# utiasSTARS/pyslam

Hardware: AMD Instinct MI355X
Metric: ms/LM-iter (Jac build + J^T J + Schur solve), stereo BA @ 500k residuals (lower is better)
Workload: dtype f64

## Files before the change

### pyslam_amd/csrc/ps_abi_problem.h

```cpp


const char* ps_last_error(void) { return g_err.c_str(); }

int ps_device_count(void) {
    int n = 0;
    if (hipGetDeviceCount(&n) != hipSuccess) return 0;
    return n;
}

int ps_warm_up(void) {
    static std::once_flag once;
    static int rc = 0;
    std::call_once(once, [] {
        void* p = nullptr;
        if (hipMalloc(&p, 256) != hipSuccess) { rc = fail("hipMalloc failed (no usable HIP device?)"); return; }
        hipLaunchKernelGGL(k_zero4, dim3(1), dim3(256), 0, 0, (size_t)8, (double*)p, (size_t)0, (double*)nullptr, (size_t)0,
                           (double*)nullptr, (size_t)0, (double*)nullptr);
        double hostw[4] = {0, 0, 0, 0};
        (void)hipMemsetAsync(p, 0, 256, 0);
        (void)hipMemcpyAsync((char*)p + 128, p, 64, hipMemcpyDeviceToDevice, 0);
        (void)hipMemcpyAsync(hostw, p, sizeof(hostw), hipMemcpyDeviceToHost, 0);
        if (hipDeviceSynchronize() != hipSuccess) rc = fail("the warm-up launch failed");
        hipFree(p);
        hipFuncAttributes a;
#define PS_TOUCH(...) (void)hipFuncGetAttributes(&a, reinterpret_cast<const void*>(&__VA_ARGS__))
        PS_TOUCH(k_landmark_pass<false>); PS_TOUCH(k_landmark_pass_packed<false, false>); PS_TOUCH(k_landmark_pass_packed<false, true>); PS_TOUCH(k_backsub_packed<false>); PS_TOUCH(k_pose_pass<false>); PS_TOUCH(k_pose_finalize); PS_TOUCH(k_schur_pairs_db<0>);
        PS_TOUCH(k_schur_combine); PS_TOUCH(k_backsub<false>); PS_TOUCH(k_cost_reproj<false>); PS_TOUCH(k_cost_packed<false>); PS_TOUCH(k_reduce3); PS_TOUCH(k_reduce_partials);
        PS_TOUCH(k_copy2); PS_TOUCH(k_zero4); PS_TOUCH(k_lag_status_check);
        PS_TOUCH(k_block_jacobi_factor<6>); PS_TOUCH(k_scale_blocks<6>); PS_TOUCH(k_scale_blocks_p<6>); PS_TOUCH(k_rows_setup<6>);
        PS_TOUCH(k_coarse_rowsums<6>); PS_TOUCH(k_coarse_matrix<6>); PS_TOUCH(k_coarse_chol<6, true>); PS_TOUCH(k_coarse_border<6>);
        PS_TOUCH(k_coarse_mreduce<6>); PS_TOUCH(k_coarse_xbuild<6>); PS_TOUCH(k_coarse_recover<6>); PS_TOUCH(k_cg_fused_lds<6, 8>);
        PS_TOUCH(k_cg_fused<6, 8>); PS_TOUCH(k_cg_unscale<6>); PS_TOUCH(k_update_poses<6>); PS_TOUCH(k_update_points);
        PS_TOUCH(k_xcoarse_rowsums<6>); PS_TOUCH(k_xcoarse_matrix<6>); PS_TOUCH(k_band_chol<6>); PS_TOUCH(k_band_inverse); PS_TOUCH(k_band_inverse_rl<false>);
        PS_TOUCH(k_band_inverse_rl<true>); PS_TOUCH(k_bp_v); PS_TOUCH(k_bp_t); PS_TOUCH(k_bp_w); PS_TOUCH(k_bp_dense_sep); PS_TOUCH(k_bp_dense);
        PS_TOUCH(k_xcg_restrict<6>); PS_TOUCH(k_xcg_f2_coarse<6, 3>); PS_TOUCH(k_xcg_fused1<6, 8, false>); PS_TOUCH(k_xcg_fused1<6, 0, true>);
        PS_TOUCH(k_xcg_fused1<6, 2, false>); PS_TOUCH(k_xcg_fused1<6, 6, false>);
        PS_TOUCH(k_factor_pass<6>); PS_TOUCH(k_factor_assemble<6>); PS_TOUCH(k_cost_factors<6>);
        PS_TOUCH(k_factor_pass<3>); PS_TOUCH(k_factor_assemble<3>); PS_TOUCH(k_cost_factors<3>); PS_TOUCH(k_block_jacobi_factor<3>);
        PS_TOUCH(k_update_poses<3>); PS_TOUCH(k_direct_solve<6>); PS_TOUCH(k_direct_solve<3>);
        PS_TOUCH(k_motion_only_solve<false>); PS_TOUCH(k_motion_only_iteration<false>);
        PS_TOUCH(k_pcg_spmv<6>); PS_TOUCH(k_pcg_spmv<3>); PS_TOUCH(k_ldi_init); PS_TOUCH(k_ldi_update); PS_TOUCH(k_ldi_gemm); PS_TOUCH(k_ldi_mirror);
        PS_TOUCH(k_ldi_ritz); PS_TOUCH(k_ldi_seed_prep); PS_TOUCH(k_ldi_fro_total); PS_TOUCH(k_ldi_pad_identity);
        PS_TOUCH(k_ldi_scaled_dense<6>); PS_TOUCH(k_ldi_sym_unscale<6>); PS_TOUCH(k_ldi_scaled_dense<3>); PS_TOUCH(k_ldi_sym_unscale<3>);
        PS_TOUCH(k_shard_pack<6>); PS_TOUCH(k_shard_unpack<6>); PS_TOUCH(k_publish); PS_TOUCH(k_cov_rhs); PS_TOUCH(k_triangulate<false>);
        PS_TOUCH(k_scale_blocks<3>); PS_TOUCH(k_rows_setup<3>); PS_TOUCH(k_coarse_rowsums<3>); PS_TOUCH(k_coarse_matrix<3>);
        PS_TOUCH(k_coarse_chol<3, true>); PS_TOUCH(k_coarse_border<3>); PS_TOUCH(k_coarse_mreduce<3>); PS_TOUCH(k_coarse_xbuild<3>);
        PS_TOUCH(k_coarse_recover<3>); PS_TOUCH(k_cg_fused_lds<3, 8>); PS_TOUCH(k_cg_unscale<3>);
#undef PS_TOUCH
    });
// ... 574 lines not shown
        row_ptr[a + 1]++;
        if (a != b) row_ptr[b + 1]++;
    }
    for (int r = 0; r < nr; ++r) row_ptr[r + 1] += row_ptr[r];
    const long nnzb_l = row_ptr[nr];
    if (nnzb_l * DD >= (1L << 31)) return fail("reduced system too large for 32-bit block offsets");
    const int nnzb = h->nnzb = (int)nnzb_l;
    col_idx.assign(nnzb, 0);
    {
        std::vector<int32_t> f2(row_ptr.begin(), row_ptr.end() - 1);
        for (uint64_t k : keys) { const int a = (int)(k >> 32), b = (int)(uint32_t)k; if (a != b) col_idx[f2[b]++] = a; }
        for (uint64_t k : keys) { const int a = (int)(k >> 32), b = (int)(uint32_t)k; col_idx[f2[a]++] = b; }
    }
    auto slot_of = [&](int a, int b) -> int {
        const int32_t* lo = col_idx.data() + row_ptr[a];
        const int32_t* hi = col_idx.data() + row_ptr[a + 1];
        const int32_t* it = std::lower_bound(lo, hi, b);
        return (it != hi && *it == b) ? (int)(it - col_idx.data()) : -1;
    };
    std::vector<int32_t> diag_slot(nr);
    for (int r = 0; r < nr; ++r) diag_slot[r] = slot_of(r, r);
    if (h->upload(&h->row_ptr, row_ptr) || h->upload(&h->col_idx, col_idx) || h->upload(&h->diag_slot, diag_slot)) return -1;
    h->red_count = (long)nnzb * DD + (long)nr * D + 2;
    if (h->alloc(&h->red, (size_t)h->red_count + ST_NWORDS / 2)) return -1;
    h->status = reinterpret_cast<int32_t*>(h->red + h->red_count);
    h->S = h->red; h->g = h->red + (size_t)nnzb * DD; h->red_cost = h->g + (size_t)nr * D;

    lap("block pattern");
    std::vector<PairItem> pitm(task_start.size());
    {
        const long nt = (long)pitm.size();
        std::atomic<int> diag{0};
        ps_parallel(ps_host_threads(nt * 16), [&](int t, int TT) {
            for (long q = nt * t / TT, e = nt * (t + 1) / TT; q < e; ++q) {
                const uint64_t key = task_keyv[q];
                const int a = (int)(key >> 32), b = (int)(uint32_t)key;
                pitm[q] = {slot_of(a, b), slot_of(b, a), task_start[q], q + 1 < nt ? task_start[q + 1] : (int32_t)npairs_l};
                if (a == b) diag = 1;
            }
        });
        if (diag) h->has_diag_tasks = true;
    }
    h->npair_items = (int)pitm.size();
    if (!dev_pairs && h->upload(&h->pairs, pairs)) return -1;
    {
        std::vector<std::vector<int32_t>> lists(8);
        const double total = (double)npairs_l;
        for (size_t k = 0; k < pitm.size(); ++k) {
// ... 193 lines not shown
```

### pyslam_amd/csrc/ps_abi_solver.h

```cpp

int ps_get_info(ps_problem* h, ps_problem_info* info) {
    if (!h || !info) return fail("null argument");
    info->dof = h->D; info->num_poses = h->P; info->num_reduced = h->nr; info->num_points = h->L;
    info->num_var_points = h->nv; info->num_obs = h->N; info->num_edges = h->F; info->num_priors = 0;
    info->reduced_nnzb = h->nnzb; info->num_pairs = h->npairs;
    info->reduce_count = ((long)h->nnzb + h->nr) / 2 * h->D * h->D + (long)h->nr * h->D + 3;
    info->device_bytes = (int64_t)h->dev_bytes;
    info->cg_restarts = h->cg_fallbacks;
    info->cg_kernel_launches = h->cg_kernel_launches;
    info->ldi_solves = h->ldi_solves; info->ldi_fallbacks = h->ldi_fallbacks; info->ldi_seeds = h->ldi_seeds;
    info->xcg_fused_solves = h->xf_solves; info->xcg_fused_fallbacks = h->xf_fallbacks;
    info->cg_persist_solves = h->cp_launches; info->cg_persist_failures = h->cp_failures;
    info->cg_persist_refused = h->cp_refused; info->persist_cus = h->persist_cus;
    info->persist_cus_needed = h->cp_ok ? h->cp_cus_needed : (h->xp_ok ? h->xp_cus_needed : 0);
    info->landmark_passes_taken_over = h->prelm_used;
    return 0;
}

int ps_eval_cost(ps_problem* h, int include_all_constant, double* cost) {
    if (!h || !cost) return fail("null argument");
    if (include_all_constant && h->fuse_cost == 1 && lm_cost_possible(h)) { if (lm_cost_pass(h, h->lin_lambda, SC_COST)) return -1; }
    else if (cost_pass(h, include_all_constant, SC_COST)) return -1;
    if (read_scalars(h)) return -1;
    *cost = h->h_scalars[SC_COST];
// ... 810 lines not shown
    if (n == "solve_horizon") { h->solve_horizon = value < 0 ? -1 : (int)std::min(value, 1e6); return 0; }
    h->prelin_valid = h->prelm_valid = false;
    if (n == "pcg_variant") { if (value != 0 && value != 1) return fail("pcg_variant must be 0 or 1"); h->pcg_variant = (int)value; }
    else if (n == "coarse_groups") {
        if (value < -1 || value >= PS_XCG_MAXNODES) return fail("coarse_groups out of range (-1 auto, 0 off, else number of hat intervals; above 63 only for the explicit two-level PCG, at most 1023)");
        h->coarse_req = (int)value; h->coarse_built = false;
    }
#ifdef PS_MEASURE
    else if (n == "cg_ablate") h->cg_ablate = (int)value;
    else if (n == "schur_ablate") h->schur_ablate = (int)value;
    else if (n == "lm_ablate") h->lm_ablate = (int)value;
#else
    else if (n == "cg_ablate" || n == "schur_ablate" || n == "lm_ablate") {
        if (value != 0.0) return fail(n + ": timing experiments exist in the measurement build only (__graft_entry__.build_measure(), PYSLAM_AMD_MEASURE=1)");
    }
#endif
    else if (n == "schur_pipeline") h->schur_pipeline = value != 0.0;
    else if (n == "coarse_lag") h->coarse_lag = value != 0.0;
    else if (n == "cg_force_restart") h->cg_force_restart = value != 0.0;
    else if (n == "xcg_restrict_fused") h->xcg_rt = value != 0;
    else if (n == "band_chol") { h->band_chol = value != 0; h->lci_next = -1; }
    else if (n == "lm_packed") h->lm_packed = value != 0;
    else if (n == "pose_xcd") h->pose_xcd = value != 0;
    else if (n == "fuse_cost") h->fuse_cost = (int)value;
    else if (n == "sync_refactor") h->sync_refactor = value != 0;
    else if (n == "hold_across_steps") h->hold_across_steps = value != 0;
    else if (n == "band_part") { h->band_part = value != 0; h->lci_next = -1; }
    else if (n == "band_part_chunk") { if (value < 0 || value > 4096) return fail("band_part_chunk must be 0 (automatic) .. 4096 nodes"); h->band_part_m = (int)value; h->lci_next = -1; }
    else if (n == "coarse_auto_hold") h->xcg_auto_hold = value != 0;
    else if (n == "coarse_adaptive_hold") h->xcg_adaptive_hold = value != 0;
    else if (n == "xcg_fused") { if (value != 0 && value != 1 && value != 2) return fail("xcg_fused must be 0, 1 or 2"); h->xcg_fused = (int)value; }
    else if (n == "lagged_inverse") { h->ldi_enable = value != 0; if (!h->ldi_enable) { h->ldi_cur = -1; if (h->ldi_state != 1) h->ldi_state = 0; } relook_path(h); }
    else if (n == "ldi_max_unknowns") { if (value < 0 || value > PS_LDI_MAXN) return fail("ldi_max_unknowns out of range (0 .. 3328)"); h->ldi_max_n = (int)value; relook_path(h); }
    else if (n == "ldi_cap") { if (value < 1 || value > 64) return fail("ldi_cap out of range (1 .. 64)"); h->ldi_cap = (int)value; }
    else if (n == "ldi_cost_tol") { if (!(value >= 0)) return fail("ldi_cost_tol must be >= 0"); h->ldi_cost_tol = value; }
    else if (n == "ldi_refresh_its") { if (value < 0 || value > 64) return fail("ldi_refresh_its out of range (0 .. 64)"); h->ldi_refresh_its = (int)value; }
    else if (n == "ldi_direct") { h->ldi_direct_ok = value != 0.0; h->ldi_direct = value > 0.0; }
    else if (n == "direct_fused") h->direct_fused = value != 0.0;
    else if (n == "ldi_seed_lag") { if (value < 1 || value > 16) return fail("ldi_seed_lag out of range (1 .. 16)"); h->ldi_seed_lag = (int)value; }
    else if (n == "ldi_seed_steps") { if (value < 1 || value > 40) return fail("ldi_seed_steps out of range (1 .. 40)"); h->ldi_seed_steps = (int)value; }
    else if (n == "coarse_refresh_every") { if (value < 1 || value > 16) return fail("coarse_refresh_every must be 1..16"); h->xcg_refresh_every = (int)value; }
    else if (n == "coarse_lag_x") { h->lagx = value != 0.0; h->lci_next = -1; h->side_todo = false; }
    else if (n == "cg_lds") h->cg_lds = value != 0.0;
    else if (n == "cg_persist") h->cg_persist = value != 0.0;
    else if (n == "xcg_persist") h->xcg_persist = value != 0.0;
    else if (n == "cg_persist_spin") { if (value < 0 || value > 1e7) return fail("cg_persist_spin out of range"); h->cp_spin = (unsigned)value; }
// ... 101 lines not shown
```

### pyslam_amd/csrc/ps_core.hip

```cpp
#include <hip/hip_runtime.h>

#include <algorithm>
#include <array>
#include <map>
#include <atomic>
#include <chrono>
#include <thread>
#include <climits>
#include <cmath>
#include <cstdio>
#include <cstring>
#include <memory>
#include <mutex>
#include <string>
#include <vector>

#include "pyslam_hip.h"
#include "ps_kernels.h"
#include "ps_ransac.h"
#include "ps_k_twoview.h"
#include "ps_photo.h"
#include "ps_k_dense.h"
#include "ps_k_feat.h"
#include "ps_sparse.h"
// ... 326 lines not shown
    typedef int (*allreduce_fn)(const void*, void*, size_t, int, int, void*, hipStream_t);
    allreduce_fn nccl_allreduce = nullptr;
    void* nccl_comm = nullptr;
    typedef int (*allgather_fn)(const void*, void*, size_t, int, void*, hipStream_t);
    allgather_fn seg_allgather = nullptr;
    int seg_world = 0, seg_rank = 0;
    long seg_maxlen = 0, seg_nmine = 0, seg_ndst = 0;
    int32_t *seg_mine = nullptr, *seg_dst = nullptr, *seg_src_off = nullptr, *seg_src_ptr = nullptr;
    double *seg_in = nullptr, *seg_all = nullptr;
    double* shard_pack = nullptr;
    int32_t *up_slot = nullptr, *upT_slot = nullptr;
    long nup = 0, pack_count = 0;
    double* shard_buf = nullptr;
    bool shard_out = false;
    double *sq_part_l = nullptr, *sq_part_p = nullptr;
    bool lm_md = false;
    double *md_part_p = nullptr, *md_part_l = nullptr;
    int nmd_p = 0;
    int nsq_l = 0 , nsq_l16 = 0 , nsq_p = 0;
    int32_t* lmw_first = nullptr;
    int lmw_nwaves = 0;
    int lm_packed = 1;
    int pose_xcd = 1;
    int ldi_enable = 1;
    int ldi_max_n = 2048;
    int ldi_cap = 12;
    int ldi_seed_steps = 3;
    double ldi_cost_tol = 0.05;
    bool ldi_ready = false;
    int ldi_n = 0, ldi_np = 0, ldi_kp = 0;
    float *ldi_S32 = nullptr, *ldi_X32 = nullptr, *ldi_R32 = nullptr, *ldi_T32 = nullptr, *ldi_Xt = nullptr, *ldi_XtT = nullptr;
    float* ldi_Xu[2] = {};
    double *ldi_x64 = nullptr, *ldi_Linv = nullptr, *ldi_r[2] = {}, *ldi_part = nullptr, *ldi_fro_part = nullptr;
    double *h_ldi_fro = nullptr, *h_ldi_fro_dev = nullptr;
    int ldi_state = 0;
    int ldi_cur = -1, ldi_next = -1;
    long ldi_iter = 0, ldi_ready_at = 0;
    double ldi_fro_limit = 0.1, ldi_last_rms = 0.0;
    bool ldi_side_todo = false, ldi_update_ok = false, ldi_sread_pending = false, ldi_ritz_ok = false;
    double ldi_ritz_lo = 0.0, ldi_ritz_hi = 0.0;
    int ldi_last_its = 0, ldi_prev_its = 0;
    int ldi_refresh_its = 7;
    bool ldi_refreshed = false;
    int2* ldi_krange = nullptr;
    int ldi_seed_lag = ps_env("PS_LDI_SEED_LAG") ? atoi(ps_env("PS_LDI_SEED_LAG")) : 1;
    int ldi_rejects = 0; long ldi_no_seed_before = 0;
// ... 168 lines not shown
```

### pyslam_amd/csrc/ps_host_cg.h

```cpp

namespace {

struct StageTimer {
    ps_problem* h;
    int stage;
    hipEvent_t a = nullptr, b = nullptr;
    int slot = -1;
    StageTimer(ps_problem* h_, int st, int level = 2) : h(h_), stage(st) {
        if (h->profiling < level) return;
        if (h->profiling == 1 && h->prof_every > 1 &&
            h->prof_tick % h->prof_every != (st == PS_ST_CG_KERNEL ? h->prof_every / 2 : 0)) return;
        if (h->ev_used + 2 > h->ev_pool.size()) {
            for (int i = 0; i < 64; ++i) { hipEvent_t e; hipEventCreate(&e); h->ev_pool.push_back(e); }
        }
        slot = (int)h->ev_used;
        a = h->ev_pool[h->ev_used++];
        b = h->ev_pool[h->ev_used++];
        hipEventRecord(a, h->stream);
    }
    void stop() {
        if (!a) return;
        hipEventRecord(b, h->stream);
        h->pending.push_back({stage, slot});
        a = nullptr;
// ... 848 lines not shown
    if (iters_out) *iters_out = total_its;
    if (relres_out) *relres_out = rel * reduced;
    h->last_pcg_iters = total_its;
    return rc;
}

int linearize(ps_problem* h, double lambda, bool allow_prelm) {
    h->solver_touched = true;
    h->prelin_valid = false;
    const bool lm_done = allow_prelm && h->prelm_valid && h->prelm_lambda == lambda && h->nv > 0;
    h->prelm_valid = false;
    h->lin_lmfail_tag = lm_done ? h->prelm_tag : 0;
    if (lm_done) ++h->prelm_used;
    h->lin_lambda = lambda;
    h->params_moved_since_lin = false; h->z_foreign = false;
    ++h->prof_tick;
    h->cov_ready = false;
    cov_release(h);
    h->status_clean = false;
    if (h->ldi_sread_pending) {
        HIP_OK(hipStreamWaitEvent(h->stream, h->ev_ldi_sread, 0));
        h->ldi_sread_pending = false;
    }
    HIP_OK(hipMemsetAsync(h->red, 0, h->red_count * sizeof(double) + ST_NWORDS * sizeof(int32_t), h->stream));
    if (h->nv > 0 && !lm_done) {
        StageTimer t(h, PS_ST_LANDMARK);
        const ObsWide wl{h->sidx_l, h->stiff_tab};
#define PS_LM_LAUNCH(W) hipLaunchKernelGGL(k_landmark_pass<W>, dim3(cdiv(h->nv, 256 / PS_LM_GROUP)), dim3(256), 0, h->stream, h->nv, h->lm_ptr, \
                           h->lm_point, h->lobs, h->poses, h->points, h->pose_rid, h->ogroups, lambda, h->Z,                       \
                           h->Cinv, h->cvec, h->status, h->lm_ablate, wl)
#define PS_LMP_LAUNCH(W) hipLaunchKernelGGL((k_landmark_pass_packed<W, false>), dim3(cdiv(h->lmw_nwaves, 4)), dim3(256), 0, h->stream, h->lmw_nwaves, \
                           h->lmw_first, h->lm_ptr, h->lm_point, h->lobs, h->poses, h->points, h->pose_rid, h->ogroups, lambda, h->Z,      \
                           h->Cinv, h->cvec, h->status, wl, (const int32_t*)nullptr, (double*)nullptr, (long long*)nullptr, 0LL)
        if (h->lm_packed && h->lmw_nwaves > 0 && !h->lm_ablate) { if (h->wide_obs) PS_LMP_LAUNCH(true); else PS_LMP_LAUNCH(false); }
        else if (h->wide_obs) PS_LM_LAUNCH(true); else PS_LM_LAUNCH(false);
#undef PS_LMP_LAUNCH
#undef PS_LM_LAUNCH
    }
    bool fin_in_combine = false, fin_in_pairs = false;
    static const bool schur_split_env = ps_env("PS_SCHUR_SPLIT") != nullptr;
    if (h->npitems > 0) {
        StageTimer t(h, PS_ST_POSE);
        const ObsWide wp{h->sidx_p, h->stiff_tab};
        const int per_xcd = h->pose_xcd ? cdiv(h->npitems, 8) : 0;
        const int nblk = per_xcd ? 8 * per_xcd : h->npitems;
        if (h->wide_obs)
            hipLaunchKernelGGL(k_pose_pass<true>, dim3(nblk), dim3(256), 0, h->stream, h->pitems, h->pobs,
                               h->poses, h->points, h->ogroups, h->Cinv, h->cvec, h->ppartial, lambda != 0.0 ? 1 : 0, wp, h->npitems, per_xcd);
        else
            hipLaunchKernelGGL(k_pose_pass<false>, dim3(nblk), dim3(256), 0, h->stream, h->pitems, h->pobs,
                               h->poses, h->points, h->ogroups, h->Cinv, h->cvec, h->ppartial, lambda != 0.0 ? 1 : 0, wp, h->npitems, per_xcd);
        fin_in_combine = h->Spart && h->npair_items > 0 && !h->has_diag_tasks && h->D == 6;
        fin_in_pairs = !h->Spart && h->schur_pipeline && h->npair_items > 0 && !h->has_diag_tasks && h->D == 6 && !schur_split_env;
        if (!fin_in_combine && !fin_in_pairs)
            hipLaunchKernelGGL(k_pose_finalize, dim3(h->nr), dim3(64), 0, h->stream, h->nr, h->pitem_ptr,
                               h->ppartial, h->diag_slot, lambda, h->S, h->g);
    }
    if (h->npair_items > 0) {
        StageTimer t(h, PS_ST_SCHUR, 1);
        const bool split2 = schur_split_env;
        const int halfp = split2 ? (h->pair_per_xcd / 2 + 3) / 4 * 4 : h->pair_per_xcd;
        static const int lds_pad = ps_env("PS_SCHUR_LDS_PAD") ? atoi(ps_env("PS_SCHUR_LDS_PAD")) : 0;
        auto launch_pairs = [&](int nblk, int lds, int from, int to) {
            if (!h->schur_pipeline)
                hipLaunchKernelGGL(k_schur_pairs, dim3(nblk), dim3(256), lds, h->stream, h->pair_per_xcd, h->pair_xitems, h->pairs,
                                   h->Z, h->S, h->Spart, h->schur_ablate, from, to);
            else {
#ifdef PS_MEASURE
                auto k = h->schur_ablate == 0 ? k_schur_pairs_db<0> : h->schur_ablate == 1 ? k_schur_pairs_db<1> :
                         h->schur_ablate == 2 ? k_schur_pairs_db<2> : h->schur_ablate == 3 ? k_schur_pairs_db<3> :
                         h->schur_ablate == 4 ? k_schur_pairs_db<4> : k_schur_pairs_db<5>;
#else
                auto k = k_schur_pairs_db<0>;
#endif
                hipLaunchKernelGGL(k, dim3(nblk + (fin_in_pairs ? cdiv(h->nr, 4) : 0)), dim3(256), lds, h->stream, h->pair_per_xcd,
                                   h->pair_xitems, h->pairs, h->Z, h->S, h->Spart, from, to, nblk, fin_in_pairs ? h->nr : 0,
                                   h->pitem_ptr, h->ppartial, h->diag_slot, lambda, h->g);
            }
        };
        launch_pairs(8 * (halfp / 4), lds_pad, 0, halfp);
        if (split2 && halfp < h->pair_per_xcd) launch_pairs(8 * ((h->pair_per_xcd - halfp + 3) / 4), 0, halfp, h->pair_per_xcd);
        if (h->Spart)
            hipLaunchKernelGGL(k_schur_combine, dim3(cdiv(h->ncomb, 4) + (fin_in_combine ? cdiv(h->nr, 4) : 0)), dim3(256), 0,
                               h->stream, h->ncomb, h->comb_items, h->comb_tasks, h->Spart, h->S,
                               fin_in_combine ? h->nr : 0, h->pitem_ptr, h->ppartial, h->diag_slot, lambda, h->g);
    }
    if ((h->F > 0 || h->FH > 0) && h->nr > 0) {
        StageTimer t(h, PS_ST_EDGES);
        if (h->D == 6) launch_factor_pass<6>(h, lambda); else launch_factor_pass<3>(h, lambda);
    }
    return side_kick(h);
}

inline bool cost_packed_possible(const ps_problem* h) {
    return h->fuse_cost != 0 && h->lm_packed && h->lmw_nwaves > 0 && !h->lm_ablate && h->Nl == h->N && h->nv > 0 && h->D == 6;
}
int cost_partials_pass(ps_problem* h, int include_all, const int32_t* gate) {
    int n = 0;
    if (h->N > 0 && include_all && cost_packed_possible(h)) {
        const ObsWide wl{h->sidx_l, h->stiff_tab};
// ... 193 lines not shown
```

### pyslam_amd/csrc/ps_k_linearize.h

```cpp
#pragma once

#define PS_LM_GROUP 16

PS_DEV double group16_sum(double v) {
    v = dpp_shift_add<0x111, 0xf, 0xf>(v);
    v = dpp_shift_add<0x112, 0xf, 0xf>(v);
    v = dpp_shift_add<0x114, 0xf, 0xe>(v);
    v = dpp_shift_add<0x118, 0xf, 0xc>(v);
    return __shfl(v, (int)(threadIdx.x & 63) | 15, 64);
}

#define PS_ZROW 16

PS_DEV void lm_emit_m(const ReprojEval& ev, double M00, double M10, double M11, double M20, double M21,
                      double M22, double* __restrict__ m) {
#pragma unroll
    for (int a = 0; a < 3; ++a) {
        const double w0 = ev.Jp[a] * ev.Jl[0] + ev.Jp[6 + a] * ev.Jl[3] + ev.Jp[12 + a] * ev.Jl[6];
        const double w1 = ev.Jp[a] * ev.Jl[1] + ev.Jp[6 + a] * ev.Jl[4] + ev.Jp[12 + a] * ev.Jl[7];
        const double w2 = ev.Jp[a] * ev.Jl[2] + ev.Jp[6 + a] * ev.Jl[5] + ev.Jp[12 + a] * ev.Jl[8];
        m[3 * a] = w0 * M00;
        m[3 * a + 1] = w0 * M10 + w1 * M11;
        m[3 * a + 2] = w0 * M20 + w1 * M21 + w2 * M22;
    }
// ... 145 lines not shown
        F[i][2] = E[i][1] * x - E[i][0] * y;
    }
    acc[0] += e[0]; acc[1] += e[1]; acc[2] += e[2]; acc[3] += F[0][0]; acc[4] += F[0][1]; acc[5] += F[0][2];
    acc[6] += e[3]; acc[7] += e[4]; acc[8] += F[1][0]; acc[9] += F[1][1]; acc[10] += F[1][2];
    acc[11] += e[5]; acc[12] += F[2][0]; acc[13] += F[2][1]; acc[14] += F[2][2];
    acc[15] += y * F[2][0] - z * F[1][0];
    acc[16] += y * F[2][1] - z * F[1][1];
    acc[17] += y * F[2][2] - z * F[1][2];
    acc[18] += z * F[0][1] - x * F[2][1];
    acc[19] += z * F[0][2] - x * F[2][2];
    acc[20] += x * F[1][2] - y * F[0][2];
}

#define PS_NPOSE_ACC 33
#ifndef PS_POSE_TRANSPOSE
#define PS_POSE_TRANSPOSE 1
#endif
typedef const __attribute__((address_space(1))) void* ps_gptr_t;
typedef __attribute__((address_space(3))) void* ps_lptr_t;

#ifndef PS_POSE_WAVES
#define PS_POSE_WAVES 3
#endif
template <bool WIDE>
__global__ __launch_bounds__(256) __attribute__((amdgpu_waves_per_eu(PS_POSE_WAVES, 8))) void k_pose_pass(
    const PItem* __restrict__ items,
    const LObs* __restrict__ pobs ,
    const double* __restrict__ poses, const double* __restrict__ points,
    const ObsGroup* __restrict__ groups, const double* __restrict__ Cinv,
    const double* __restrict__ cvec, double* __restrict__ partial, int want_diag ,
    ObsWide wide, int nitems, int per_xcd )
{
    __shared__ double red[4][PS_NPOSE_ACC];
#if PS_POSE_TRANSPOSE
    __shared__ double tr[4][64 * 17];
#endif
    const int item = per_xcd > 0 ? (int)(blockIdx.x & 7) * per_xcd + (int)(blockIdx.x >> 3) : (int)blockIdx.x;
    if (item >= nitems) return;
    const PItem it = items[item];
    const int w = threadIdx.x >> 6, lane = threadIdx.x & 63;
    const Se3 T = se3_load(poses + 12 * (size_t)it.pad);
    double acc[PS_NPOSE_ACC];
#pragma unroll
    for (int k = 0; k < PS_NPOSE_ACC; ++k) acc[k] = 0.0;
    for (int i = it.start + threadIdx.x; i < it.end; i += 256) {
        const LObs o = pobs[i];
        const int v = PS_POSE_OF(o) - 1;
        const double pw[3] = {points[3 * (size_t)o.point], points[3 * (size_t)o.point + 1], points[3 * (size_t)o.point + 2]};
        double m[6] = {0, 0, 0, 0, 0, 0}, c0 = 0.0, c1 = 0.0, c2 = 0.0;
        if (v >= 0) {
            const double* ci = Cinv + 6 * (size_t)v;
#pragma unroll
            for (int k = 0; k < 6; ++k) m[k] = ci[k];
            c0 = cvec[3 * (size_t)v]; c1 = cvec[3 * (size_t)v + 1]; c2 = cvec[3 * (size_t)v + 2];
        }
        ReprojEval ev;
        reproj_eval_obs<true, true, WIDE>(T, pw, &o.u, groups, PS_GRP_OF(o), wide, i, ev);
        double G[6], t3[3];
        {
            const double* J = ev.Jp;
            G[0] = J[0] * J[0] + J[6] * J[6] + J[12] * J[12];
// ... 12 lines not shown
            pose_sandwich(G, ev.pc, d21);
            acc[27] += d21[0]; acc[28] += d21[6]; acc[29] += d21[11]; acc[30] += d21[15]; acc[31] += d21[18]; acc[32] += d21[20];
        }
        if (v >= 0) {
            double m9[9];
            lm_emit_m(ev, m[0], m[1], m[2], m[3], m[4], m[5], m9);
            G[0] -= m9[0] * m9[0] + m9[1] * m9[1] + m9[2] * m9[2];
            G[1] -= m9[0] * m9[3] + m9[1] * m9[4] + m9[2] * m9[5];
            G[2] -= m9[0] * m9[6] + m9[1] * m9[7] + m9[2] * m9[8];
            G[3] -= m9[3] * m9[3] + m9[4] * m9[4] + m9[5] * m9[5];
            G[4] -= m9[3] * m9[6] + m9[4] * m9[7] + m9[5] * m9[8];
            G[5] -= m9[6] * m9[6] + m9[7] * m9[7] + m9[8] * m9[8];
#pragma unroll
            for (int a = 0; a < 3; ++a) t3[a] += m9[3 * a] * c0 + m9[3 * a + 1] * c1 + m9[3 * a + 2] * c2;
        }
        pose_sandwich(G, ev.pc, acc);
        acc[21] -= t3[0]; acc[22] -= t3[1]; acc[23] -= t3[2];
        acc[24] -= ev.pc[1] * t3[2] - ev.pc[2] * t3[1];
        acc[25] -= ev.pc[2] * t3[0] - ev.pc[0] * t3[2];
        acc[26] -= ev.pc[0] * t3[1] - ev.pc[1] * t3[0];
    }
#if PS_POSE_TRANSPOSE
    {
        double* trw = tr[w];
#pragma unroll
        for (int h2 = 0; h2 < 2; ++h2) {
            const int k0 = 17 * h2, nk = h2 ? PS_NPOSE_ACC - 17 : 17;
#pragma unroll
            for (int k = 0; k < 17; ++k) if (k < nk) trw[lane * 17 + k] = acc[k0 + k];
            __builtin_amdgcn_wave_barrier();
            if (lane < nk) {
                double s = 0.0;
#pragma unroll 8
                for (int l = 0; l < 64; ++l) s += trw[l * 17 + lane];
                red[w][k0 + lane] = s;
            }
            __builtin_amdgcn_wave_barrier();
        }
    }
#else
#pragma unroll
    for (int k = 0; k < PS_NPOSE_ACC; ++k) {
        const double s = wave_sum(acc[k]);
        if (lane == 0) red[w][k] = s;
    }
#endif
    __syncthreads();
    if (threadIdx.x < PS_NPOSE_ACC)
        partial[(size_t)item * PS_NPOSE_ACC + threadIdx.x] =
            ((red[0][threadIdx.x] + red[1][threadIdx.x]) + red[2][threadIdx.x]) + red[3][threadIdx.x];
}

PS_DEV void pose_finalize_wave(int rid, int lane, const int32_t* __restrict__ pitem_ptr,
                               const double* __restrict__ partial, const int32_t* __restrict__ diag_slot,
                               double lambda, double* __restrict__ S, double* __restrict__ g, double* v )
{
    if (lane < PS_NPOSE_ACC) {
        double s = 0.0;
        for (int it = pitem_ptr[rid]; it < pitem_ptr[rid + 1]; ++it) s += partial[(size_t)it * PS_NPOSE_ACC + lane];
        v[lane] = s;
    }
    __builtin_amdgcn_wave_barrier();
    if (lane < 36) {
        const int r = lane / 6, c = lane % 6;
        const int a = r < c ? r : c, b = r < c ? c : r;
        const int idx = a * 6 - (a * (a - 1)) / 2 + (b - a);
        double val = v[idx];
        if (r == c) val += lambda * v[27 + r];
        S[(size_t)diag_slot[rid] * 36 + lane] += val;
    }
    if (lane < 6) g[(size_t)rid * 6 + lane] += v[21 + lane];
}

// ... 268 lines not shown
```

### pyslam_amd/csrc/ps_k_schur2.h

```cpp
#pragma once

#define PS_SQ_ROWD 12
#define PS_SQ_BUF (64 * PS_SQ_ROWD)
#define PS_SQ_BUFSTEP (4 * PS_SQ_BUF * 8)

typedef double ps_d2 __attribute__((ext_vector_type(2)));
#ifndef PS_SQ_ASM_CLOBBER
#define PS_SQ_ASM_CLOBBER "memory"
#endif

PS_DEV void sq_fetch_idx(const int32_t* __restrict__ src , int32_t* slot ) {
    __builtin_amdgcn_global_load_lds((ps_gptr_t)src, (ps_lptr_t)slot, 4, 0, 0);
}

template <bool HOT >
PS_DEV void sq_fetch(const double* __restrict__ Z, const uint32_t (&ia)[6], uint32_t slot_off, double* buf, const int (&off_of)[6]) {
    int zr[6];
    asm volatile(
        "ds_read_b32 %0, %6\n\t"
        "ds_read_b32 %1, %7\n\t"
        "ds_read_b32 %2, %8\n\t"
        "ds_read_b32 %3, %9\n\t"
        "ds_read_b32 %4, %10\n\t"
        "ds_read_b32 %5, %11\n\t"
// ... 38 lines not shown
#pragma unroll
        for (int k = 0; k < 9; ++k) A[k] = hf ? A[k] : ma[k];
    }
    double mb[12];
#pragma unroll
    for (int k = 0; k < 6; ++k) { mb[2 * k] = vb[k].x; mb[2 * k + 1] = vb[k].y; }
#pragma unroll
    for (int a = 0; a < 3; ++a)
#pragma unroll
        for (int b = 0; b < 3; ++b)
            acc[6 * a + b] += A[3 * a] * mb[3 * b] + A[3 * a + 1] * mb[3 * b + 1] + A[3 * a + 2] * mb[3 * b + 2];
    double Lb[9];
    zrow_cross(mb, mb + 9, Lb);
#pragma unroll
    for (int a = 0; a < 3; ++a)
#pragma unroll
        for (int b = 0; b < 3; ++b)
            acc[6 * a + 3 + b] += A[3 * a] * Lb[3 * b] + A[3 * a + 1] * Lb[3 * b + 1] + A[3 * a + 2] * Lb[3 * b + 2];
}

#define PS_SQ_WAIT_CHUNK() __builtin_amdgcn_s_waitcnt(0x0F70 | 7)
#define PS_SQ_WAIT_ALL() __builtin_amdgcn_s_waitcnt(0x0F70)

template <int ABL >
__global__ __launch_bounds__(256) __attribute__((amdgpu_waves_per_eu(3, 3))) void k_schur_pairs_db(
    int per_xcd, const PairItem* __restrict__ xitems, const int2* __restrict__ pairs, const double* __restrict__ Z,
    double* __restrict__ S, double* __restrict__ Spart, int first, int last,
    int fin_first_block, int fin_nr, const int32_t* __restrict__ pitem_ptr, const double* __restrict__ ppartial,
    const int32_t* __restrict__ diag_slot, double lambda, double* __restrict__ g)
{
    constexpr int ablate = ABL;
    __shared__ __attribute__((aligned(16))) double sbuf[2 * 4 * PS_SQ_BUF];
    __shared__ __attribute__((aligned(16))) int32_t sidx[4 * 256];
    const int lane = threadIdx.x & 63, wv = threadIdx.x >> 6;
    double* const buf0 = sbuf + wv * PS_SQ_BUF;
    double* const buf1 = buf0 + 4 * PS_SQ_BUF;
    int32_t* const islot = sidx + wv * 256;
    if ((int)blockIdx.x >= fin_first_block) {
        const int rid = ((int)blockIdx.x - fin_first_block) * 4 + wv;
        if (rid < fin_nr) pose_finalize_wave(rid, lane, pitem_ptr, ppartial, diag_slot, lambda, S, g, buf0);
        return;
    }
    const int local = first + (blockIdx.x >> 3) * 4 + wv;
    if (local >= last) return;
    const size_t pos = (size_t)(blockIdx.x & 7) * per_xcd + local;
    PairItem it = xitems[pos];
    it.slot = __builtin_amdgcn_readfirstlane(it.slot); it.slotT = __builtin_amdgcn_readfirstlane(it.slotT);
    it.start = __builtin_amdgcn_readfirstlane(it.start); it.end = __builtin_amdgcn_readfirstlane(it.end);
    if (it.slot < 0) return;
    const int p = lane & 31, hf = lane >> 5;
    const int32_t* flat = reinterpret_cast<const int32_t*>(pairs) + hf;
    uint32_t ia[6];
    int off_of[6];
#pragma unroll
    for (int k = 0; k < 6; ++k) {
        const int q = 64 * k + lane, row = q / 6;
        ia[k] = (uint32_t)(uintptr_t)(ps_lptr_t)(islot + row);
        off_of[k] = 2 * (q - 6 * row);
    }
    const uint32_t aa = (uint32_t)(uintptr_t)(ps_lptr_t)(buf0 + PS_SQ_ROWD * p), ab = aa + 32 * PS_SQ_ROWD * 8;
    double acc[18];
#pragma unroll
    for (int k = 0; k < 18; ++k) acc[k] = 0.0;
    const int npairs = it.end - it.start, nch = (npairs + 31) >> 5, last_pair = max(it.end - 1, 0);
#define PS_SQ_IDX(c) (flat + 2 * (size_t)min(it.start + 32 * (c) + p, last_pair))
    sq_fetch_idx(PS_SQ_IDX(0), islot + 0);
    sq_fetch_idx(PS_SQ_IDX(1), islot + 64);
    sq_fetch_idx(PS_SQ_IDX(2), islot + 128);
    PS_SQ_WAIT_ALL();
    __builtin_amdgcn_wave_barrier();
    if (!(ablate & 2)) sq_fetch<(ABL & 4) != 0>(Z, ia, 0, buf0, off_of);
    sq_fetch_idx(PS_SQ_IDX(3), islot + 192);
    if (nch > 1 && !(ablate & 2)) sq_fetch<(ABL & 4) != 0>(Z, ia, 256, buf1, off_of);
    int c = 0;
    for (; c + 2 < nch; ++c) {
        const uint32_t boff = (c & 1) * PS_SQ_BUFSTEP;
        PS_SQ_WAIT_CHUNK();
        __builtin_amdgcn_wave_barrier();
        if (!(ablate & 1)) sq_products(aa + boff, ab + boff, hf, acc);
        __builtin_amdgcn_wave_barrier();
        sq_fetch_idx(PS_SQ_IDX(c + 4), islot + 64 * (c & 3));
        if (!(ablate & 2)) sq_fetch<(ABL & 4) != 0>(Z, ia, 256 * ((c + 2) & 3), (c & 1) ? buf1 : buf0, off_of);
    }
    if (c + 1 < nch) {
        PS_SQ_WAIT_CHUNK();
        __builtin_amdgcn_wave_barrier();
        if (!(ablate & 1)) sq_products(aa + (c & 1) * PS_SQ_BUFSTEP, ab + (c & 1) * PS_SQ_BUFSTEP, hf, acc);
        __builtin_amdgcn_wave_barrier();
        ++c;
    }
    {
        PS_SQ_WAIT_ALL();
        __builtin_amdgcn_wave_barrier();
        if (p < npairs - 32 * c && !(ablate & 1)) sq_products(aa + (c & 1) * PS_SQ_BUFSTEP, ab + (c & 1) * PS_SQ_BUFSTEP, hf, acc);
        __builtin_amdgcn_wave_barrier();
    }
#undef PS_SQ_IDX
    double* sums = buf0;
#pragma unroll
    for (int k = 0; k < 18; ++k) {
        const double t = half_sum_dpp(acc[k]);
        if (p == 31) sums[18 * hf + k] = t;
    }
    __builtin_amdgcn_wave_barrier();
    if (lane < 36) {
// ... 13 lines not shown
```

### pyslam_amd/csrc/ps_kernels.h

```cpp
#pragma once
#include "ps_math.h"

struct __attribute__((aligned(32))) LObs {
    double u, v, d;
    int32_t pose_grp;
    int32_t point;
};
struct PItem { int32_t rid, start, end, pad; };
struct PairItem { int32_t slot, slotT, start, end; };
struct FactorGroup { double S[36]; int32_t loss_id; int32_t pad; double loss_k; };

#define PS_POSE_OF(o) ((o).pose_grp & 0xFFFFFF)
#define PS_GRP_OF(o) (((uint32_t)(o).pose_grp) >> 24)

enum { ST_LM_FAIL = 0, ST_DIAG_FAIL = 1, ST_PCG_DONE = 2, ST_PCG_ITERS = 3, ST_PERSIST_FAIL = 4 , ST_NWORDS = 8 };
enum { SC_COST = 0, SC_DXP2 = 1, SC_LINCOST = 2, SC_RR0 = 3, SC_RRFINAL = 4, SC_THRESH = 5, SC_DXL2 = 6, SC_STARTCOST = 7, SC_MODELDEC = 8, SC_NWORDS = 9 };

template <int CTRL, int ROW_MASK, int BANK_MASK>
PS_DEV double dpp_shift_add(double v) {
    const unsigned long long b = __builtin_bit_cast(unsigned long long, v);
    const int lo = __builtin_amdgcn_update_dpp(0, (int)(unsigned)b, CTRL, ROW_MASK, BANK_MASK, false);
    const int hi = __builtin_amdgcn_update_dpp(0, (int)(unsigned)(b >> 32), CTRL, ROW_MASK, BANK_MASK, false);
    const unsigned long long m = ((unsigned long long)(unsigned)hi << 32) | (unsigned)lo;
    return v + __builtin_bit_cast(double, m);
// ... 52 lines not shown
```

Baseline: 0.3062.

## Merge pose linearization pass into Schur pair kernel with atomic arrival finalize

Pose-pass workgroups now run inside the Schur pair kernel launch, reusing its LDS. The last workgroup to finish a pose row, detected through a per-row atomic arrival counter, runs the pose finalize for that row. This removes one kernel launch and the stream serialization between the pose pass and the pair pass, letting the two phases overlap. In exchange it adds atomics, memory fences and an extra zeroed counter array, and the pose work may now compete with the pair work for occupancy under the pair kernel's waves-per-EU limit.

```diff
diff --git a/pyslam_amd/csrc/ps_abi_problem.h b/pyslam_amd/csrc/ps_abi_problem.h
--- a/pyslam_amd/csrc/ps_abi_problem.h
+++ b/pyslam_amd/csrc/ps_abi_problem.h
@@ -24,7 +24,7 @@
         hipFree(p);
         hipFuncAttributes a;
 #define PS_TOUCH(...) (void)hipFuncGetAttributes(&a, reinterpret_cast<const void*>(&__VA_ARGS__))
-        PS_TOUCH(k_landmark_pass<false>); PS_TOUCH(k_landmark_pass_packed<false, false>); PS_TOUCH(k_landmark_pass_packed<false, true>); PS_TOUCH(k_backsub_packed<false>); PS_TOUCH(k_pose_pass<false>); PS_TOUCH(k_pose_finalize); PS_TOUCH(k_schur_pairs_db<0>);
+        PS_TOUCH(k_landmark_pass<false>); PS_TOUCH(k_landmark_pass_packed<false, false>); PS_TOUCH(k_landmark_pass_packed<false, true>); PS_TOUCH(k_backsub_packed<false>); PS_TOUCH(k_pose_pass<false>); PS_TOUCH(k_pose_finalize); PS_TOUCH(k_schur_pairs_db<0>); PS_TOUCH(k_schur_pairs_db<8>);
         PS_TOUCH(k_schur_combine); PS_TOUCH(k_backsub<false>); PS_TOUCH(k_cost_reproj<false>); PS_TOUCH(k_cost_packed<false>); PS_TOUCH(k_reduce3); PS_TOUCH(k_reduce_partials);
         PS_TOUCH(k_copy2); PS_TOUCH(k_zero4); PS_TOUCH(k_lag_status_check);
         PS_TOUCH(k_block_jacobi_factor<6>); PS_TOUCH(k_scale_blocks<6>); PS_TOUCH(k_scale_blocks_p<6>); PS_TOUCH(k_rows_setup<6>);
@@ -645,8 +645,9 @@
     for (int r = 0; r < nr; ++r) diag_slot[r] = slot_of(r, r);
     if (h->upload(&h->row_ptr, row_ptr) || h->upload(&h->col_idx, col_idx) || h->upload(&h->diag_slot, diag_slot)) return -1;
     h->red_count = (long)nnzb * DD + (long)nr * D + 2;
-    if (h->alloc(&h->red, (size_t)h->red_count + ST_NWORDS / 2)) return -1;
+    if (h->alloc(&h->red, (size_t)h->red_count + ST_NWORDS / 2 + ((size_t)nr + 1) / 2)) return -1;
     h->status = reinterpret_cast<int32_t*>(h->red + h->red_count);
+    h->pose_arrive = h->status + ST_NWORDS;
     h->S = h->red; h->g = h->red + (size_t)nnzb * DD; h->red_cost = h->g + (size_t)nr * D;
 
     lap("block pattern");
diff --git a/pyslam_amd/csrc/ps_abi_solver.h b/pyslam_amd/csrc/ps_abi_solver.h
--- a/pyslam_amd/csrc/ps_abi_solver.h
+++ b/pyslam_amd/csrc/ps_abi_solver.h
@@ -856,6 +856,8 @@
     else if (n == "band_chol") { h->band_chol = value != 0; h->lci_next = -1; }
     else if (n == "lm_packed") h->lm_packed = value != 0;
     else if (n == "pose_xcd") h->pose_xcd = value != 0;
+    else if (n == "lin_merged") h->lin_merged = value != 0;
+    else if (n == "lin_merged_place") { if (value != 0 && value != 1 && value != 2) return fail("lin_merged_place must be 0 (pose workgroups first), 1 (last) or 2 (interleaved)"); h->lin_merged_place = (int)value; }
     else if (n == "fuse_cost") h->fuse_cost = (int)value;
     else if (n == "sync_refactor") h->sync_refactor = value != 0;
     else if (n == "hold_across_steps") h->hold_across_steps = value != 0;
diff --git a/pyslam_amd/csrc/ps_core.hip b/pyslam_amd/csrc/ps_core.hip
--- a/pyslam_amd/csrc/ps_core.hip
+++ b/pyslam_amd/csrc/ps_core.hip
@@ -372,6 +372,8 @@
     int lmw_nwaves = 0;
     int lm_packed = 1;
     int pose_xcd = 1;
+    int lin_merged = PS_LIN_MERGED_DEFAULT, lin_merged_place = PS_LIN_MERGED_PLACE_DEFAULT;
+    int32_t* pose_arrive = nullptr;
     int ldi_enable = 1;
     int ldi_max_n = 2048;
     int ldi_cap = 12;
diff --git a/pyslam_amd/csrc/ps_host_cg.h b/pyslam_amd/csrc/ps_host_cg.h
--- a/pyslam_amd/csrc/ps_host_cg.h
+++ b/pyslam_amd/csrc/ps_host_cg.h
@@ -894,7 +894,7 @@
         HIP_OK(hipStreamWaitEvent(h->stream, h->ev_ldi_sread, 0));
         h->ldi_sread_pending = false;
     }
-    HIP_OK(hipMemsetAsync(h->red, 0, h->red_count * sizeof(double) + ST_NWORDS * sizeof(int32_t), h->stream));
+    HIP_OK(hipMemsetAsync(h->red, 0, h->red_count * sizeof(double) + (ST_NWORDS + (size_t)h->nr) * sizeof(int32_t), h->stream));
     if (h->nv > 0 && !lm_done) {
         StageTimer t(h, PS_ST_LANDMARK);
         const ObsWide wl{h->sidx_l, h->stiff_tab};
@@ -909,24 +909,33 @@
 #undef PS_LMP_LAUNCH
 #undef PS_LM_LAUNCH
     }
-    bool fin_in_combine = false, fin_in_pairs = false;
+    bool fin_in_combine = false, fin_in_pairs = false, merged = false;
     static const bool schur_split_env = ps_env("PS_SCHUR_SPLIT") != nullptr;
+    PoseMerge pm{};
     if (h->npitems > 0) {
-        StageTimer t(h, PS_ST_POSE);
         const ObsWide wp{h->sidx_p, h->stiff_tab};
         const int per_xcd = h->pose_xcd ? cdiv(h->npitems, 8) : 0;
         const int nblk = per_xcd ? 8 * per_xcd : h->npitems;
-        if (h->wide_obs)
-            hipLaunchKernelGGL(k_pose_pass<true>, dim3(nblk), dim3(256), 0, h->stream, h->pitems, h->pobs,
-                               h->poses, h->points, h->ogroups, h->Cinv, h->cvec, h->ppartial, lambda != 0.0 ? 1 : 0, wp, h->npitems, per_xcd);
-        else
-            hipLaunchKernelGGL(k_pose_pass<false>, dim3(nblk), dim3(256), 0, h->stream, h->pitems, h->pobs,
-                               h->poses, h->points, h->ogroups, h->Cinv, h->cvec, h->ppartial, lambda != 0.0 ? 1 : 0, wp, h->npitems, per_xcd);
         fin_in_combine = h->Spart && h->npair_items > 0 && !h->has_diag_tasks && h->D == 6;
         fin_in_pairs = !h->Spart && h->schur_pipeline && h->npair_items > 0 && !h->has_diag_tasks && h->D == 6 && !schur_split_env;
-        if (!fin_in_combine && !fin_in_pairs)
-            hipLaunchKernelGGL(k_pose_finalize, dim3(h->nr), dim3(64), 0, h->stream, h->nr, h->pitem_ptr,
-                               h->ppartial, h->diag_slot, lambda, h->S, h->g);
+        merged = fin_in_pairs && h->lin_merged;
+#ifdef PS_MEASURE
+        if (h->schur_ablate) merged = false;
+#endif
+        if (merged) {
+            pm = PoseMerge{wp, lambda != 0.0 ? 1 : 0, h->npitems, per_xcd, cdiv(h->npitems, 8), h->pair_per_xcd / 4, h->lin_merged_place};
+        } else {
+            StageTimer t(h, PS_ST_POSE);
+            if (h->wide_obs)
+                hipLaunchKernelGGL(k_pose_pass<true>, dim3(nblk), dim3(256), 0, h->stream, h->pitems, h->pobs,
+                                   h->poses, h->points, h->ogroups, h->Cinv, h->cvec, h->ppartial, lambda != 0.0 ? 1 : 0, wp, h->npitems, per_xcd);
+            else
+                hipLaunchKernelGGL(k_pose_pass<false>, dim3(nblk), dim3(256), 0, h->stream, h->pitems, h->pobs,
+                                   h->poses, h->points, h->ogroups, h->Cinv, h->cvec, h->ppartial, lambda != 0.0 ? 1 : 0, wp, h->npitems, per_xcd);
+            if (!fin_in_combine && !fin_in_pairs)
+                hipLaunchKernelGGL(k_pose_finalize, dim3(h->nr), dim3(64), 0, h->stream, h->nr, h->pitem_ptr,
+                                   h->ppartial, h->diag_slot, lambda, h->S, h->g);
+        }
     }
     if (h->npair_items > 0) {
         StageTimer t(h, PS_ST_SCHUR, 1);
@@ -945,9 +954,17 @@
 #else
                 auto k = k_schur_pairs_db<0>;
 #endif
+                if (merged) {
+                    k = h->wide_obs ? k_schur_pairs_db<24> : k_schur_pairs_db<8>;
+                    hipLaunchKernelGGL(k, dim3(8 * ps_linm_rows(pm.rows, pm.pair_rows)), dim3(256), lds, h->stream, h->pair_per_xcd,
+                                       h->pair_xitems, h->pairs, h->Z, h->S, h->Spart, from, to, 0, 0,
+                                       h->pitem_ptr, h->ppartial, h->diag_slot, lambda, h->g, pm, h->pitems, h->pobs, h->poses,
+                                   h->points, h->ogroups, h->Cinv, h->cvec, h->ppartial, h->pose_arrive);
+                } else
                 hipLaunchKernelGGL(k, dim3(nblk + (fin_in_pairs ? cdiv(h->nr, 4) : 0)), dim3(256), lds, h->stream, h->pair_per_xcd,
                                    h->pair_xitems, h->pairs, h->Z, h->S, h->Spart, from, to, nblk, fin_in_pairs ? h->nr : 0,
-                                   h->pitem_ptr, h->ppartial, h->diag_slot, lambda, h->g);
+                                   h->pitem_ptr, h->ppartial, h->diag_slot, lambda, h->g, pm, h->pitems, h->pobs, h->poses,
+                                   h->points, h->ogroups, h->Cinv, h->cvec, h->ppartial, h->pose_arrive);
             }
         };
         launch_pairs(8 * (halfp / 4), lds_pad, 0, halfp);
diff --git a/pyslam_amd/csrc/ps_k_linearize.h b/pyslam_amd/csrc/ps_k_linearize.h
--- a/pyslam_amd/csrc/ps_k_linearize.h
+++ b/pyslam_amd/csrc/ps_k_linearize.h
@@ -191,21 +191,16 @@
 #ifndef PS_POSE_WAVES
 #define PS_POSE_WAVES 3
 #endif
+#define PS_POSE_TR_DOUBLES (4 * 64 * 17)
 template <bool WIDE>
-__global__ __launch_bounds__(256) __attribute__((amdgpu_waves_per_eu(PS_POSE_WAVES, 8))) void k_pose_pass(
-    const PItem* __restrict__ items,
+PS_DEV void pose_pass_item(
+    int item, const PItem* __restrict__ items,
     const LObs* __restrict__ pobs ,
     const double* __restrict__ poses, const double* __restrict__ points,
     const ObsGroup* __restrict__ groups, const double* __restrict__ Cinv,
-    const double* __restrict__ cvec, double* __restrict__ partial, int want_diag ,
-    ObsWide wide, int nitems, int per_xcd )
-{
-    __shared__ double red[4][PS_NPOSE_ACC];
-#if PS_POSE_TRANSPOSE
-    __shared__ double tr[4][64 * 17];
-#endif
-    const int item = per_xcd > 0 ? (int)(blockIdx.x & 7) * per_xcd + (int)(blockIdx.x >> 3) : (int)blockIdx.x;
-    if (item >= nitems) return;
+    const double* __restrict__ cvec, double* partial, int want_diag ,
+    const ObsWide& wide, double (*red)[PS_NPOSE_ACC], double* trbase, bool sc1 = false )
+{
     const PItem it = items[item];
     const int w = threadIdx.x >> 6, lane = threadIdx.x & 63;
     const Se3 T = se3_load(poses + 12 * (size_t)it.pad);
@@ -264,7 +259,7 @@
     }
 #if PS_POSE_TRANSPOSE
     {
-        double* trw = tr[w];
+        double* trw = trbase + w * (64 * 17);
 #pragma unroll
         for (int h2 = 0; h2 < 2; ++h2) {
             const int k0 = 17 * h2, nk = h2 ? PS_NPOSE_ACC - 17 : 17;
@@ -288,9 +283,29 @@
     }
 #endif
     __syncthreads();
-    if (threadIdx.x < PS_NPOSE_ACC)
-        partial[(size_t)item * PS_NPOSE_ACC + threadIdx.x] =
-            ((red[0][threadIdx.x] + red[1][threadIdx.x]) + red[2][threadIdx.x]) + red[3][threadIdx.x];
+    if (threadIdx.x < PS_NPOSE_ACC) {
+        const double sum = ((red[0][threadIdx.x] + red[1][threadIdx.x]) + red[2][threadIdx.x]) + red[3][threadIdx.x];
+        if (sc1) __hip_atomic_store(&partial[(size_t)item * PS_NPOSE_ACC + threadIdx.x], sum, __ATOMIC_RELAXED, __HIP_MEMORY_SCOPE_AGENT);
+        else partial[(size_t)item * PS_NPOSE_ACC + threadIdx.x] = sum;
+    }
+}
+
+template <bool WIDE>
+__global__ __launch_bounds__(256) __attribute__((amdgpu_waves_per_eu(PS_POSE_WAVES, 8))) void k_pose_pass(
+    const PItem* __restrict__ items, const LObs* __restrict__ pobs, const double* __restrict__ poses, const double* __restrict__ points,
+    const ObsGroup* __restrict__ groups, const double* __restrict__ Cinv,
+    const double* __restrict__ cvec, double* __restrict__ partial, int want_diag,
+    ObsWide wide, int nitems, int per_xcd )
+{
+    __shared__ double red[4][PS_NPOSE_ACC];
+#if PS_POSE_TRANSPOSE
+    __shared__ double tr[PS_POSE_TR_DOUBLES];
+#else
+    double* const tr = nullptr;
+#endif
+    const int item = ps_linm_pose_item((int)blockIdx.x, per_xcd);
+    if (item >= nitems) return;
+    pose_pass_item<WIDE>(item, items, pobs, poses, points, groups, Cinv, cvec, partial, want_diag, wide, red, tr);
 }
 
 PS_DEV void pose_finalize_wave(int rid, int lane, const int32_t* __restrict__ pitem_ptr,
diff --git a/pyslam_amd/csrc/ps_k_schur2.h b/pyslam_amd/csrc/ps_k_schur2.h
--- a/pyslam_amd/csrc/ps_k_schur2.h
+++ b/pyslam_amd/csrc/ps_k_schur2.h
@@ -84,28 +84,63 @@
 #define PS_SQ_WAIT_CHUNK() __builtin_amdgcn_s_waitcnt(0x0F70 | 7)
 #define PS_SQ_WAIT_ALL() __builtin_amdgcn_s_waitcnt(0x0F70)
 
+struct PoseMerge {
+    ObsWide wide;
+    int want_diag, nitems, per_xcd;
+    int rows, pair_rows, placement;
+};
+
 template <int ABL >
 __global__ __launch_bounds__(256) __attribute__((amdgpu_waves_per_eu(3, 3))) void k_schur_pairs_db(
     int per_xcd, const PairItem* __restrict__ xitems, const int2* __restrict__ pairs, const double* __restrict__ Z,
     double* __restrict__ S, double* __restrict__ Spart, int first, int last,
     int fin_first_block, int fin_nr, const int32_t* __restrict__ pitem_ptr, const double* __restrict__ ppartial,
-    const int32_t* __restrict__ diag_slot, double lambda, double* __restrict__ g)
+    const int32_t* __restrict__ diag_slot, double lambda, double* __restrict__ g,
+    PoseMerge pm, const PItem* __restrict__ items, const LObs* __restrict__ pobs, const double* __restrict__ poses,
+    const double* __restrict__ points, const ObsGroup* __restrict__ groups, const double* __restrict__ Cinv,
+    const double* __restrict__ cvec, double* mpartial, int32_t* arrive)
 {
-    constexpr int ablate = ABL;
+    constexpr int ablate = ABL & 7;
+    constexpr bool MERGED = (ABL & 8) != 0;
     __shared__ __attribute__((aligned(16))) double sbuf[2 * 4 * PS_SQ_BUF];
     __shared__ __attribute__((aligned(16))) int32_t sidx[4 * 256];
+    static_assert(sizeof(sbuf) >= PS_POSE_TR_DOUBLES * sizeof(double) && sizeof(sidx) >= 4 * PS_NPOSE_ACC * sizeof(double),
+                  "the pose workgroups reduce in the pair workgroups' LDS");
     const int lane = threadIdx.x & 63, wv = threadIdx.x >> 6;
     double* const buf0 = sbuf + wv * PS_SQ_BUF;
     double* const buf1 = buf0 + 4 * PS_SQ_BUF;
     int32_t* const islot = sidx + wv * 256;
-    if ((int)blockIdx.x >= fin_first_block) {
+    int bx = (int)blockIdx.x;
+    if (MERGED) {
+        int idx;
+        const bool pose_row = ps_linm_role((int)(blockIdx.x >> 3), pm.rows, pm.pair_rows, pm.placement, &idx) != 0;
+        bx = 8 * idx + (int)(blockIdx.x & 7);
+        if (pose_row) {
+            const int item = ps_linm_pose_item(bx, pm.per_xcd);
+            if (item >= pm.nitems) return;
+            pose_pass_item<(ABL & 16) != 0>(item, items, pobs, poses, points, groups, Cinv, cvec, mpartial, pm.want_diag,
+                                            pm.wide, reinterpret_cast<double (*)[PS_NPOSE_ACC]>(sidx), sbuf, true);
+            if (wv != 0) return;
+            const int rid = __builtin_amdgcn_readfirstlane(items[item].rid);
+            const int nit = pitem_ptr[rid + 1] - pitem_ptr[rid];
+            asm volatile("s_waitcnt vmcnt(0)" ::: "memory");
+            int prev = 0;
+            if (lane == 0) prev = __hip_atomic_fetch_add(arrive + rid, 1, __ATOMIC_RELAXED, __HIP_MEMORY_SCOPE_AGENT);
+            prev = __builtin_amdgcn_readfirstlane(prev);
+            if (prev != nit - 1) return;
+            __builtin_amdgcn_fence(__ATOMIC_ACQUIRE, "agent");
+            asm volatile("s_waitcnt vmcnt(0)" ::: "memory");
+            pose_finalize_wave(rid, lane, pitem_ptr, mpartial, diag_slot, lambda, S, g, sbuf);
+            return;
+        }
+    } else if ((int)blockIdx.x >= fin_first_block) {
         const int rid = ((int)blockIdx.x - fin_first_block) * 4 + wv;
         if (rid < fin_nr) pose_finalize_wave(rid, lane, pitem_ptr, ppartial, diag_slot, lambda, S, g, buf0);
         return;
     }
-    const int local = first + (blockIdx.x >> 3) * 4 + wv;
+    const int local = first + (bx >> 3) * 4 + wv;
     if (local >= last) return;
-    const size_t pos = (size_t)(blockIdx.x & 7) * per_xcd + local;
+    const size_t pos = (size_t)(bx & 7) * per_xcd + local;
     PairItem it = xitems[pos];
     it.slot = __builtin_amdgcn_readfirstlane(it.slot); it.slotT = __builtin_amdgcn_readfirstlane(it.slotT);
     it.start = __builtin_amdgcn_readfirstlane(it.start); it.end = __builtin_amdgcn_readfirstlane(it.end);
@@ -131,9 +166,9 @@
     sq_fetch_idx(PS_SQ_IDX(2), islot + 128);
     PS_SQ_WAIT_ALL();
     __builtin_amdgcn_wave_barrier();
-    if (!(ablate & 2)) sq_fetch<(ABL & 4) != 0>(Z, ia, 0, buf0, off_of);
+    if (!(ablate & 2)) sq_fetch<(ablate & 4) != 0>(Z, ia, 0, buf0, off_of);
     sq_fetch_idx(PS_SQ_IDX(3), islot + 192);
-    if (nch > 1 && !(ablate & 2)) sq_fetch<(ABL & 4) != 0>(Z, ia, 256, buf1, off_of);
+    if (nch > 1 && !(ablate & 2)) sq_fetch<(ablate & 4) != 0>(Z, ia, 256, buf1, off_of);
     int c = 0;
     for (; c + 2 < nch; ++c) {
         const uint32_t boff = (c & 1) * PS_SQ_BUFSTEP;
@@ -142,7 +177,7 @@
         if (!(ablate & 1)) sq_products(aa + boff, ab + boff, hf, acc);
         __builtin_amdgcn_wave_barrier();
         sq_fetch_idx(PS_SQ_IDX(c + 4), islot + 64 * (c & 3));
-        if (!(ablate & 2)) sq_fetch<(ABL & 4) != 0>(Z, ia, 256 * ((c + 2) & 3), (c & 1) ? buf1 : buf0, off_of);
+        if (!(ablate & 2)) sq_fetch<(ablate & 4) != 0>(Z, ia, 256 * ((c + 2) & 3), (c & 1) ? buf1 : buf0, off_of);
     }
     if (c + 1 < nch) {
         PS_SQ_WAIT_CHUNK();
diff --git a/pyslam_amd/csrc/ps_kernels.h b/pyslam_amd/csrc/ps_kernels.h
--- a/pyslam_amd/csrc/ps_kernels.h
+++ b/pyslam_amd/csrc/ps_kernels.h
@@ -1,5 +1,6 @@
 #pragma once
 #include "ps_math.h"
+#include "ps_lin_merged.h"
 
 struct __attribute__((aligned(32))) LObs {
     double u, v, d;
diff --git a/pyslam_amd/csrc/ps_lin_merged.h b/pyslam_amd/csrc/ps_lin_merged.h
--- /dev/null
+++ b/pyslam_amd/csrc/ps_lin_merged.h
@@ -0,0 +1,45 @@
+#ifndef PS_LIN_MERGED_H
+#define PS_LIN_MERGED_H
+
+#ifndef PS_HD
+#if defined(__HIPCC__)
+#define PS_HD __host__ __device__
+#else
+#define PS_HD
+#endif
+#endif
+
+enum { PS_LINM_POSE_FIRST = 0, PS_LINM_POSE_LAST = 1, PS_LINM_INTERLEAVED = 2, PS_LINM_NPLACE = 3 };
+
+#ifndef PS_LIN_MERGED_DEFAULT
+#define PS_LIN_MERGED_DEFAULT 1
+#endif
+#ifndef PS_LIN_MERGED_PLACE_DEFAULT
+#define PS_LIN_MERGED_PLACE_DEFAULT PS_LINM_POSE_LAST
+#endif
+
+PS_HD static inline int ps_linm_rows(int rp, int rq) { return rp + rq; }
+
+PS_HD static inline int ps_linm_role(int row, int rp, int rq, int placement, int* idx) {
+    if (placement == PS_LINM_POSE_FIRST) {
+        if (row < rp) { *idx = row; return 1; }
+        *idx = row - rp;
+        return 0;
+    }
+    if (placement == PS_LINM_POSE_LAST) {
+        if (row < rq) { *idx = row; return 0; }
+        *idx = row - rq;
+        return 1;
+    }
+    {
+        const long long n = (long long)rp + rq;
+        const int before = (int)((long long)row * rp / n), upto = (int)(((long long)row + 1) * rp / n);
+        if (upto > before) { *idx = before; return 1; }
+        *idx = row - before;
+        return 0;
+    }
+}
+
+PS_HD static inline int ps_linm_pose_item(int pb, int per_xcd) { return per_xcd > 0 ? (pb & 7) * per_xcd + (pb >> 3) : pb; }
+
+#endif
```

New measurement: 0.3043 (median of 4 runs). No clear change (-0.6%).
